# parsakhaz/multimodal-image-similarity-search

Measured on AMD Instinct MI355X. Metric: images/s CLIP-B/32 encode @ bs256; Mvec/s cosine top-10 over 10M x 512, higher is better.
Workload: dtype bf16

## Files before the change

### multimodal-image-similarity-search_amd/csrc/gemm_bf16_p160.h

```cpp
#pragma once
#include "gemm_bf16_256.h"

#define MMISS_EPI_PATCH_PIX_F32 10

#define G160_A_BYTES 20480
#define G160_W_BYTES 16384
#define G160_BUF (G160_A_BYTES + 2 * G160_W_BYTES)
#define G160_DUMP (3 * G160_BUF)
#define G160_LDS (G160_DUMP + 2048)

template <int EPI, int KT = 0>
__global__ __launch_bounds__(512, 2) void gemm160p_kernel(const __bf16* __restrict__ A, const __bf16* __restrict__ W, int M,
                                                          int N, int K, GemmEpi ep) {
    extern __shared__ __attribute__((aligned(16))) char smem[];
    typedef bf16x8 frag;
    const int tid = threadIdx.x;
    const int lane = tid & 63;
    const int wave = __builtin_amdgcn_readfirstlane(tid >> 6);
    const int wm = wave >> 2, wn = wave & 3;
    const int fr = lane & 15, fg = lane >> 4;
    const int nbm = M / 160, nbn = N >> 8;
    const int nt = KT > 0 ? KT : K / GEMM_BK;
    const int wg = xcd_remap(blockIdx.x, nbm * nbn);
    int bm, bn;
    tile_order(wg, nbm, nbn, 0, bm, bn);
    const __bf16* Ab = A + (size_t)bm * 160 * K;
    const __bf16* Wb = W + (size_t)bn * 256 * K;

    constexpr bool RESID = (EPI == MMISS_EPI_BIAS_RESID_BF16);
    constexpr bool PIX = (EPI == MMISS_EPI_PATCH_PIX_F32);
    constexpr bool PATCH = (EPI == MMISS_EPI_PATCH_F32) || PIX;
    static_assert(RESID || PATCH, "gemm160p_kernel: epilogue");
    const int r_in = lane >> 3, p = lane & 7;
    int lane_vo = (r_in * K + ((p ^ r_in) * 8)) * 2;
    __amdgpu_buffer_rsrc_t srdA = __builtin_amdgcn_make_buffer_rsrc(const_cast<__bf16*>(Ab), 0, 0x7fffffff, 0x00020000);
    __amdgpu_buffer_rsrc_t srdW = __builtin_amdgcn_make_buffer_rsrc(const_cast<__bf16*>(Wb), 0, 0x7fffffff, 0x00020000);
    const int row8 = 8 * K * 2;
    const int a_so = wave * row8;
    const int a_dst = wave * 1024;
    const int w_so = ((wave >> 1) * 64 + (wave & 1) * 16) * K * 2;
    const int w_dst = wave * 2048;
    int xa0 = a_so, xa1 = a_so + 8 * row8, xa2 = a_so + 16 * row8, xaf = a_so;
    int xw0 = w_so, xw1 = w_so + row8, xw2 = w_so + 4 * row8, xw3 = w_so + 5 * row8;
    int kstep = GEMM_BK * 2;
#define G160_X(var, expr) (RESID ? (var) : (expr))
    char* const dump = smem + G160_DUMP + wave * 256;
#define G160_BLDS(srd, so, dst) \
    __builtin_amdgcn_raw_ptr_buffer_load_lds(srd, (__attribute__((address_space(3))) void*)(dst), 16, lane_vo, so, 0, 0)
#define G160_FILL(srd, so) \
    __builtin_amdgcn_raw_ptr_buffer_load_lds(srd, (__attribute__((address_space(3))) void*)(dump), 4, lane_vo, so, 0, 0)
#define G160_STAGE_A(b2, ko)                                                                                 \
    {                                                                                                       \
        char* sl_ = smem + (b2) * G160_BUF + a_dst;                                                         \
        G160_BLDS(srdA, G160_X(xa0, a_so) + (ko), sl_);                                                     \
        G160_BLDS(srdA, G160_X(xa1, a_so + 8 * row8) + (ko), sl_ + 8 * 1024);                               \
        if (wave < 4) { G160_BLDS(srdA, G160_X(xa2, a_so + 16 * row8) + (ko), sl_ + 16 * 1024); }           \
        else { G160_FILL(srdA, G160_X(xaf, a_so) + (ko)); }                                                 \
    }
#define G160_STAGE_W(b2, nq, ko)                                                                             \
    {                                                                                                       \
        char* sl_ = smem + (b2) * G160_BUF + G160_A_BYTES + (nq) * G160_W_BYTES + w_dst;                    \
        const int so_ = G160_X((nq) ? xw2 : xw0, w_so + (nq) * 4 * row8) + (ko);                            \
        G160_BLDS(srdW, so_, sl_);                                                                          \
        G160_BLDS(srdW, G160_X(((nq) ? xw3 : xw1) + (ko), so_ + row8), sl_ + 1024);                         \
    }

    const int rblk = 16 * ep.ldo * 2;
    const int lane_vo_r = ((lane >> 2) * ep.ldo + (((lane & 3) ^ (lane >> 4)) * 8)) * 2;
#define G160_NEXT_KTILE()                                                                                    \
    if (++k2 == nt) {                                                                                       \
        if constexpr (RESID) {                                                                              \
            srdA = srdW = __builtin_amdgcn_make_buffer_rsrc(                                                \
                reinterpret_cast<uint16_t*>(ep.out) + (size_t)(bm * 160 + wm * 80) * ep.ldo + bn * 256 + wn * 64, 0, 0x7fffffff, \
                0x00020000);                                                                                \
            lane_vo = lane_vo_r;                                                                            \
            xa0 = 0; xa1 = 64; xa2 = 0; xaf = 0;                                                            \
            xw0 = rblk; xw1 = rblk + 64; xw2 = 2 * rblk; xw3 = 2 * rblk + 64;                               \
            ko2 = 0; kstep = 2 * rblk;                                                                      \
        } else { k2 = 0; ko2 = 0; }                                                                         \
    } else { ko2 += kstep; }

    u32x4 srdP = {0u, 0u, 0u, 0u};
    int pvo[3] = {0, 0, 0};
    u32x4 pa[2][6];
    int pix_S = 0, pix_tshift = 0, pix_rows = 0, pix_half = 0;
    if constexpr (PIX) {
        const uint64_t a64 = (uint64_t)A;
        srdP = u32x4{(uint32_t)a64, (uint32_t)(a64 >> 32) & 0xffffu, (uint32_t)ep.pix_bytes, 0x00020000u};
        const int S = ep.pix_S, P = ep.pix_P, G = S / P, GG = ep.p0;
        pix_S = S;
        pix_tshift = P == 32 ? 4 : 2;
        pix_rows = 64 / P;
        const int dky = P == 32 ? 0 : (p >> 2), kx = P == 32 ? p * 4 : (p & 3) * 4;
        pix_half = (P == 32 ? 1 : 2) * S * 4;
#pragma unroll
        for (int j = 0; j < 3; ++j) {
            const int q = wave + 8 * ((j == 2 && wave >= 4) ? 1 : j);
            int m = bm * 160 + q * 8 + r_in;
            m = m < ep.m_valid ? m : ep.m_valid - 1;
            const int img = m / GG, pr = m - img * GG, py = pr / G, px = pr - py * G;
            pvo[j] = (((img * 3) * S + py * P + dky) * S + px * P + kx) * 4;
        }
    }
#define G160_PIX_LOAD(set, kt)                                                                               \
    {                                                                                                       \
        const int c_ = (kt) >> pix_tshift;                                                                  \
        const int so_ = (c_ * pix_S + ((kt) - (c_ << pix_tshift)) * pix_rows) * pix_S * 4;                  \
        const int so2_ = so_ + pix_half;                                                                    \
        _Pragma("unroll") for (int j = 0; j < 3; ++j)                                                       \
            asm volatile("buffer_load_dwordx4 %0, %2, %3, %4 offen\n\tbuffer_load_dwordx4 %1, %2, %3, %5 offen" \
                         : "=&v"(pa[set][2 * j]), "=&v"(pa[set][2 * j + 1])                                 \
                         : "v"(pvo[j]), "s"(srdP), "s"(so_), "s"(so2_)                                      \
                         : "memory");                                                                       \
    }
#define G160_PIX_WRITE(set, b2, cnt)                                                                         \
    {                                                                                                       \
        asm volatile("s_waitcnt vmcnt(" #cnt ")"                                                            \
                     : "+v"(pa[set][0]), "+v"(pa[set][1]), "+v"(pa[set][2]), "+v"(pa[set][3]), "+v"(pa[set][4]), "+v"(pa[set][5]) \
                     :: "memory");                                                                          \
         \
        const int ao_ = (b2) * G160_BUF + a_dst + r_in * 128 + (((p >> 1) ^ r_in) << 4) + ((p & 1) << 3);   \
        _Pragma("unroll") for (int j = 0; j < 3; ++j) {                                                     \
            const u32x4 lo_ = pa[set][2 * j], hi_ = pa[set][2 * j + 1];                                     \
            u32x2 pl_, ph_;                                                                                 \
            pl_[0] = pack_bf16x2(__uint_as_float(lo_[0]), __uint_as_float(lo_[1]));                         \
            pl_[1] = pack_bf16x2(__uint_as_float(lo_[2]), __uint_as_float(lo_[3]));                         \
            ph_[0] = pack_bf16x2(__uint_as_float(hi_[0]), __uint_as_float(hi_[1]));                         \
            ph_[1] = pack_bf16x2(__uint_as_float(hi_[2]), __uint_as_float(hi_[3]));                         \
            if (j < 2 || wave < 4) {                                                                        \
                *reinterpret_cast<u32x2*>(smem + ao_ + j * 8 * 1024) = pl_;                                 \
                *reinterpret_cast<u32x2*>(smem + (ao_ ^ 64) + j * 8 * 1024) = ph_;                          \
            }                                                                                               \
        }                                                                                                   \
    }

    uint32_t ab[2], wb[2];
#pragma unroll
    for (int s = 0; s < 2; ++s) {
        const uint32_t sw = (((4 * s + fg) ^ (fr & 7)) << 4);
        ab[s] = (wm * 80 + fr) * 128 + sw;
        wb[s] = G160_A_BYTES + (wn * 32 + fr) * 128 + sw;
    }
    frag am[5];
    frag wq[4];
    f32x4 acc[4][5];
#pragma unroll
    for (int i = 0; i < 4; ++i)
#pragma unroll
        for (int j = 0; j < 5; ++j) acc[i][j] = f32x4{0.f, 0.f, 0.f, 0.f};

#define G160_READ(b, s)                                                                                      \
    {                                                                                                       \
        _Pragma("unroll") for (int mf = 0; mf < 5; ++mf)                                                    \
            am[mf] = *reinterpret_cast<const frag*>(smem + ab[s] + (b) * G160_BUF + mf * 2048);             \
        _Pragma("unroll") for (int i = 0; i < 4; ++i)                                                       \
            wq[i] = *reinterpret_cast<const frag*>(smem + wb[s] + (b) * G160_BUF + (i >> 1) * G160_W_BYTES + (i & 1) * 2048); \
    }
#define G160_MMA()                                                                                           \
    {                                                                                                       \
        __builtin_amdgcn_s_setprio(1);                                                                      \
        _Pragma("unroll") for (int i = 0; i < 4; ++i)                                                       \
            _Pragma("unroll") for (int mf = 0; mf < 5; ++mf)                                                \
                acc[i][mf] = __builtin_amdgcn_mfma_f32_16x16x32_bf16(wq[i], am[mf], acc[i][mf], 0, 0, 0);   \
        __builtin_amdgcn_s_setprio(0);                                                                      \
    }
#define G160_KTILE(B, B2)                                                                                    \
    {                                                                                                       \
        G160_READ(B, 0);                                                                                    \
        G160_STAGE_A(B2, ko2);                                                                              \
        p256s_late_reads_done(wm);                                                                             \
        p256s_barrier();                                                                                     \
        G160_MMA();                                                                                         \
        p256s_barrier();                                                                                     \
        G160_READ(B, 1);                                                                                    \
        G160_STAGE_W(B2, 0, ko2);                                                                           \
        G160_STAGE_W(B2, 1, ko2);                                                                           \
        p256s_late_reads_done(wm);                                                                             \
        asm volatile("s_waitcnt vmcnt(7)" ::: "memory");                                                    \
        p256s_barrier();                                                                                     \
        G160_MMA();                                                                                         \
        p256s_barrier();                                                                                     \
        G160_NEXT_KTILE();                                                                                  \
    }

#define G160_KTILE_PIX(B, B1, B2, SET)                                                                       \
    {                                                                                                       \
        G160_READ(B, 0);                                                                                    \
        G160_PIX_LOAD(SET, k2);                                                                             \
        p256s_late_reads_done(wm);                                                                             \
        p256s_barrier();                                                                                     \
        G160_MMA();                                                                                         \
        p256s_barrier();                                                                                     \
        G160_READ(B, 1);                                                                                    \
        G160_PIX_WRITE((SET) ^ 1, B1, 10);                                                                  \
        G160_STAGE_W(B2, 0, ko2);                                                                           \
        G160_STAGE_W(B2, 1, ko2);                                                                           \
        asm volatile("s_waitcnt vmcnt(10) lgkmcnt(0)" ::: "memory");                                        \
        p256s_barrier();                                                                                     \
        G160_MMA();                                                                                         \
        p256s_barrier();                                                                                     \
        G160_NEXT_KTILE();                                                                                  \
    }

    f32x4 bias[4];
    if constexpr (RESID) {
#pragma unroll
        for (int i = 0; i < 4; ++i) bias[i] = *reinterpret_cast<const f32x4*>(ep.bias + bn * 256 + wn * 64 + i * 16 + 4 * fg);
    }

    int ko2 = 0, k2 = 2;
    if constexpr (PIX) {
        G160_PIX_LOAD(0, 0);
        G160_STAGE_W(0, 0, 0);
        G160_STAGE_W(0, 1, 0);
        G160_PIX_LOAD(1, 1);
        G160_STAGE_W(1, 0, GEMM_BK * 2);
        G160_STAGE_W(1, 1, GEMM_BK * 2);
        G160_PIX_WRITE(0, 0, 14);
        ko2 = 2 * GEMM_BK * 2;
        asm volatile("s_waitcnt vmcnt(10) lgkmcnt(0)" ::: "memory");
    } else {
    G160_STAGE_A(0, 0);
    G160_STAGE_W(0, 0, 0);
    G160_STAGE_W(0, 1, 0);
    G160_STAGE_A(1, GEMM_BK * 2);
    G160_STAGE_W(1, 0, GEMM_BK * 2);
    G160_STAGE_W(1, 1, GEMM_BK * 2);
    ko2 = (nt > 2) ? 2 * GEMM_BK * 2 : 0;
    asm volatile("s_waitcnt vmcnt(7)" ::: "memory");
    }
    if constexpr (RESID) {
#pragma unroll
        for (int i = 0; i < 4; ++i) asm volatile("" : "+v"(bias[i]));
    }
    p256s_barrier();
    if (wm == 1) p256s_barrier();

    if constexpr (PIX) {
#pragma unroll 1
        for (int t = 0; t < nt; t += 6) {
            G160_KTILE_PIX(0, 1, 2, 0);
            G160_KTILE_PIX(1, 2, 0, 1);
            G160_KTILE_PIX(2, 0, 1, 0);
            G160_KTILE_PIX(0, 1, 2, 1);
            G160_KTILE_PIX(1, 2, 0, 0);
            G160_KTILE_PIX(2, 0, 1, 1);
        }
    } else {
#pragma unroll 1
    for (int t = 0; t < nt; t += 3) {
        G160_KTILE(0, 2);
        if (t + 1 < nt) G160_KTILE(1, 0);
        if (t + 2 < nt) G160_KTILE(2, 1);
    }
    }
    if (wm == 0) p256s_barrier();
    asm volatile("s_waitcnt vmcnt(0)" ::: "memory");
    p256s_barrier();
    const int free_buf = RESID ? ((nt + 2) % 3) * G160_BUF : 0;

    if constexpr (PATCH) {
        int lane_e = lane;
        asm volatile("" : "+v"(lane_e));
        const int efr = lane_e & 15, efg = lane_e >> 4;
        const int rrow = lane_e >> 3, rchunk = lane_e & 7;
        char* patch = smem + free_buf + wave * 2048;
        float* outp = reinterpret_cast<float*>(ep.out);
#pragma unroll
        for (int j = 0; j < 5; ++j) {
#pragma unroll
            for (int h = 0; h < 2; ++h) {
#pragma unroll
                for (int ii = 0; ii < 2; ++ii)
                    *reinterpret_cast<f32x4*>(patch + efr * 128 + (((ii * 4 + efg) ^ (efr & 7)) << 4)) = acc[2 * h + ii][j];
                __builtin_amdgcn_fence(__ATOMIC_RELEASE, "wavefront");
                __builtin_amdgcn_wave_barrier();
                __builtin_amdgcn_fence(__ATOMIC_ACQUIRE, "wavefront");
#pragma unroll
                for (int rh = 0; rh < 2; ++rh) {
                    const int row = rh * 8 + rrow;
                    const f32x4 v = *reinterpret_cast<const f32x4*>(patch + row * 128 + ((rchunk ^ (row & 7)) << 4));
                    const int m = bm * 160 + wm * 80 + j * 16 + row;
                    const int n = bn * 256 + wn * 64 + h * 32 + rchunk * 4;
                    if (m < ep.m_valid) {
                        const int img = m / ep.p0, pt = m - img * ep.p0;
                        const f32x4 pos = *reinterpret_cast<const f32x4*>(ep.aux + (size_t)(1 + pt) * ep.ldo + n);
                        *reinterpret_cast<f32x4*>(outp + ((size_t)img * ep.p1 + 1 + pt) * ep.ldo + n) = v + pos;
                    }
                }
                __builtin_amdgcn_wave_barrier();
            }
        }
    }
    if constexpr (RESID) {
        int lane_e = lane;
        asm volatile("" : "+v"(lane_e));
        const int efr = lane_e & 15, efg = lane_e >> 4;
        const int rrow = lane_e >> 3, rchunk = lane_e & 7;
        const __amdgpu_buffer_rsrc_t srdO = __builtin_amdgcn_make_buffer_rsrc(ep.out, 0, 0x7fffffff, 0x00020000);
        char* patch = smem + free_buf + wave * 2048;
        const int wr_off = efr * 128, wr_sw = 2 * (efr & 7);
        const int col = bn * 256 + wn * 64 + rchunk * 8;
        const int dump_row = M - 1;
        u32x2 resid[5][4];
        {
            const char* const st0 = smem + (nt % 3) * G160_BUF;
            const char* const st1 = smem + ((nt + 1) % 3) * G160_BUF;
            const int rd = efr * 64 + ((((efg >> 1) ^ (efr >> 2)) << 4) | ((efg & 1) << 3));
#pragma unroll
            for (int j = 0; j < 5; ++j)
#pragma unroll
                for (int i = 0; i < 4; ++i) {
                    const int h = i >> 1;
                    const char* piece = j == 0 ? st0 + a_dst + h * 8 * 1024
                                               : (j < 3 ? st0 : st1) + G160_A_BYTES + ((j - 1) & 1) * G160_W_BYTES + w_dst + h * 1024;
                    resid[j][i] = *reinterpret_cast<const u32x2*>(piece + (rd ^ ((i & 1) << 5)));
                }
        }
#pragma unroll
        for (int j = 0; j < 5; ++j) {
#pragma unroll
            for (int i = 0; i < 4; ++i) {
                const f32x4 v = acc[i][j] + bias[i];
                float y[4];
                y[0] = __uint_as_float(resid[j][i][0] << 16) + v[0];
                y[1] = __uint_as_float(resid[j][i][0] & 0xFFFF0000u) + v[1];
                y[2] = __uint_as_float(resid[j][i][1] << 16) + v[2];
                y[3] = __uint_as_float(resid[j][i][1] & 0xFFFF0000u) + v[3];
                u32x2 pk;
                pk[0] = pack_bf16x2(y[0], y[1]);
                pk[1] = pack_bf16x2(y[2], y[3]);
                *reinterpret_cast<u32x2*>(patch + wr_off + (((i * 4 + efg) ^ wr_sw) << 3)) = pk;
            }
            __builtin_amdgcn_fence(__ATOMIC_RELEASE, "wavefront");
            __builtin_amdgcn_wave_barrier();
            __builtin_amdgcn_fence(__ATOMIC_ACQUIRE, "wavefront");
#pragma unroll
            for (int rh = 0; rh < 2; ++rh) {
                const int row = rh * 8 + rrow;
                const u32x4 pk = *reinterpret_cast<const u32x4*>(patch + row * 128 + (((2 * rchunk) ^ (2 * (row & 7))) << 3));
                const int m = bm * 160 + wm * 80 + j * 16 + row;
                const int vo = ((m < ep.m_valid ? m : dump_row) * ep.ldo + col) * 2;
                __builtin_amdgcn_raw_buffer_store_b128(pk, srdO, vo, 0, 0);
                if (ep.stats_out) {
                    float rs = 0.f, rq = 0.f;
#pragma unroll
                    for (int e = 0; e < 4; ++e) {
                        const float a = __uint_as_float(pk[e] << 16), b = __uint_as_float(pk[e] & 0xFFFF0000u);
                        rs += a + b;
                        rq += a * a + b * b;
                    }
                    rs += __shfl_xor(rs, 1); rq += __shfl_xor(rq, 1);
                    rs += __shfl_xor(rs, 2); rq += __shfl_xor(rq, 2);
                    rs += __shfl_xor(rs, 4); rq += __shfl_xor(rq, 4);
                    if (rchunk == 0 && m < ep.m_valid) {
                        float* so = ep.stats_out + ((size_t)m * (ep.ldo >> 6) + ((bn * 256 + wn * 64) >> 6)) * 2;
                        so[0] = rs;
                        so[1] = rq;
                    }
                }
            }
            __builtin_amdgcn_wave_barrier();
        }
    }
}
#undef G160_BLDS
#undef G160_FILL
#undef G160_STAGE_A
#undef G160_STAGE_W
#undef G160_READ
#undef G160_MMA
#undef G160_KTILE
#undef G160_KTILE_PIX
#undef G160_PIX_LOAD
#undef G160_PIX_WRITE
#undef G160_NEXT_KTILE
#undef G160_X

static inline bool gemm160p_ok(int M, int N, int K) {
    if (M <= 0 || (M % 160) || N <= 0 || (N % 256) || K < 256 || (K % 128)) return false;
    if ((int64_t)M * N * 2 >= (1LL << 31) || (int64_t)160 * K * 2 >= (1LL << 31) || (int64_t)256 * K * 2 >= (1LL << 31)) return false;
    return true;
}

static int launch_gemm160p(hipStream_t st, const void* A, const void* W, const GemmEpi& ep, int M, int N, int K) {
    if (!gemm160p_ok(M, N, K)) MM_FAIL(MMISS_ERR_UNSUPPORTED, "gemm160p: M=%d N=%d K=%d", M, N, K);
    if (!ep.out || !ep.bias || ep.ldo < N || (ep.ldo % 64)) MM_FAIL(MMISS_ERR_ARG, "gemm160p: missing operand");
    const int mv = ep.m_valid < M ? ep.m_valid : M;
    const double bytes = 2.0 * ((double)mv * K + (double)N * K) + 2.0 * 2.0 * (double)mv * N;
    char pname[48];
    snprintf(pname, sizeof(pname), "gemm_bf16_bias_resid16_p160_k%d", K);
    MM_PROF(pname, st, 2.0 * mv * N * K, bytes);
#define G160_KT_CASE(KT_)                                                                                                        \
    if (K == (KT_) * GEMM_BK) {                                                                                                  \
        MM_TRY(mmiss_ensure_dyn_lds(reinterpret_cast<const void*>(&gemm160p_kernel<MMISS_EPI_BIAS_RESID_BF16, KT_>), G160_LDS)); \
        hipLaunchKernelGGL((gemm160p_kernel<MMISS_EPI_BIAS_RESID_BF16, KT_>), dim3((M / 160) * (N / 256)), dim3(512), G160_LDS, \
                           st, reinterpret_cast<const __bf16*>(A), reinterpret_cast<const __bf16*>(W), M, N, K, ep);            \
        MM_HIP(hipGetLastError());                                                                                              \
        return MMISS_OK;                                                                                                        \
    }
    G160_KT_CASE(12) G160_KT_CASE(48) G160_KT_CASE(8) G160_KT_CASE(32) G160_KT_CASE(16) G160_KT_CASE(64)
#undef G160_KT_CASE
    MM_TRY(mmiss_ensure_dyn_lds(reinterpret_cast<const void*>(&gemm160p_kernel<MMISS_EPI_BIAS_RESID_BF16>), G160_LDS));
    hipLaunchKernelGGL((gemm160p_kernel<MMISS_EPI_BIAS_RESID_BF16>), dim3((M / 160) * (N / 256)), dim3(512), G160_LDS, st, reinterpret_cast<const __bf16*>(A),
                       reinterpret_cast<const __bf16*>(W), M, N, K, ep);
    MM_HIP(hipGetLastError());
    return MMISS_OK;
}

static int launch_gemm160p_patch(hipStream_t st, const void* A, const void* W, const GemmEpi& ep, int M, int N, int K) {
    if (!gemm160p_ok(M, N, K)) MM_FAIL(MMISS_ERR_UNSUPPORTED, "gemm160p_patch: M=%d N=%d K=%d", M, N, K);
    if (!ep.out || !ep.aux || ep.p0 <= 0 || ep.p1 <= 0 || ep.ldo < N) MM_FAIL(MMISS_ERR_ARG, "gemm160p_patch: missing operand");
    const int mv = ep.m_valid < M ? ep.m_valid : M;
    MM_PROF("gemm_bf16_patch_p160", st, 2.0 * mv * N * K, 2.0 * ((double)mv * K + (double)N * K) + 4.0 * (double)mv * N);
    MM_TRY(mmiss_ensure_dyn_lds(reinterpret_cast<const void*>(&gemm160p_kernel<MMISS_EPI_PATCH_F32>), G160_LDS));
    hipLaunchKernelGGL((gemm160p_kernel<MMISS_EPI_PATCH_F32>), dim3((M / 160) * (N / 256)), dim3(512), G160_LDS, st,
                       reinterpret_cast<const __bf16*>(A), reinterpret_cast<const __bf16*>(W), M, N, K, ep);
    MM_HIP(hipGetLastError());
    return MMISS_OK;
}

static inline bool gemm160p_pix_ok(const void* pixels, int B, int S, int P, int M, int N, int K) {
    if (!(P == 16 || P == 32) || S <= 0 || (S % P) || K != 3 * P * P || !gemm160p_ok(M, N, K)) return false;
    const int G = S / P;
    if ((int64_t)B * G * G > M || ((uintptr_t)pixels & 15)) return false;
    return (int64_t)B * 3 * S * S * 4 < (1LL << 31);
}
static int launch_gemm160p_patch_pix(hipStream_t st, const void* pixels, const void* W, const GemmEpi& ep0, int B, int S, int P, int M,
                                     int N, int K) {
    if (!gemm160p_pix_ok(pixels, B, S, P, M, N, K)) MM_FAIL(MMISS_ERR_UNSUPPORTED, "gemm160p_patch_pix: B=%d S=%d P=%d M=%d N=%d K=%d", B, S, P, M, N, K);
    GemmEpi ep = ep0;
    const int G = S / P;
    if (!ep.out || !ep.aux || ep.p0 != G * G || ep.p1 <= 0 || ep.ldo < N || ep.m_valid != B * G * G)
        MM_FAIL(MMISS_ERR_ARG, "gemm160p_patch_pix: missing operand");
    ep.pix_S = S; ep.pix_P = P; ep.pix_bytes = (int)((int64_t)B * 3 * S * S * 4);
    const int mv = ep.m_valid;
    MM_PROF("gemm_bf16_patch_p160", st, 2.0 * mv * N * K, 4.0 * (double)B * 3 * S * S + 2.0 * (double)N * K + 4.0 * (double)mv * N);
    MM_TRY(mmiss_ensure_dyn_lds(reinterpret_cast<const void*>(&gemm160p_kernel<MMISS_EPI_PATCH_PIX_F32>), G160_LDS));
    hipLaunchKernelGGL((gemm160p_kernel<MMISS_EPI_PATCH_PIX_F32>), dim3((M / 160) * (N / 256)), dim3(512), G160_LDS, st,
                       reinterpret_cast<const __bf16*>(pixels), reinterpret_cast<const __bf16*>(W), M, N, K, ep);
    MM_HIP(hipGetLastError());
    return MMISS_OK;
}
```

Before: 92460.

## Pipeline residual GEMM epilogue with double-buffered patch and DPP row reductions

```diff
diff --git a/multimodal-image-similarity-search_amd/csrc/gemm_bf16_p160.h b/multimodal-image-similarity-search_amd/csrc/gemm_bf16_p160.h
--- a/multimodal-image-similarity-search_amd/csrc/gemm_bf16_p160.h
+++ b/multimodal-image-similarity-search_amd/csrc/gemm_bf16_p160.h
@@ -8,6 +8,29 @@
 #define G160_BUF (G160_A_BYTES + 2 * G160_W_BYTES)
 #define G160_DUMP (3 * G160_BUF)
 #define G160_LDS (G160_DUMP + 2048)
+
+__device__ __forceinline__ void g160_row_sum8(float& a, float& b, float& c, float& d) {
+#define G160_DPP4(ctrl)                                              \
+    "v_add_f32_dpp %0, %0, %0 " ctrl " row_mask:0xf bank_mask:0xf\n\t" \
+    "v_add_f32_dpp %1, %1, %1 " ctrl " row_mask:0xf bank_mask:0xf\n\t" \
+    "v_add_f32_dpp %2, %2, %2 " ctrl " row_mask:0xf bank_mask:0xf\n\t" \
+    "v_add_f32_dpp %3, %3, %3 " ctrl " row_mask:0xf bank_mask:0xf\n\t"
+    asm("s_nop 1\n\t" G160_DPP4("quad_perm:[1,0,3,2]") G160_DPP4("quad_perm:[2,3,0,1]") G160_DPP4("row_half_mirror")
+        : "+v"(a), "+v"(b), "+v"(c), "+v"(d));
+#undef G160_DPP4
+}
+
+__device__ __forceinline__ void g160_row_part(const u32x4& pk, float& rs, float& rq) {
+#pragma clang fp contract(off)
+    rs = 0.f;
+    rq = 0.f;
+#pragma unroll
+    for (int e = 0; e < 4; ++e) {
+        const float a = __uint_as_float(pk[e] << 16), b = __uint_as_float(pk[e] & 0xFFFF0000u);
+        rs += a + b;
+        rq += a * a + b * b;
+    }
+}
 
 template <int EPI, int KT = 0>
 __global__ __launch_bounds__(512, 2) void gemm160p_kernel(const __bf16* __restrict__ A, const __bf16* __restrict__ W, int M,
@@ -255,16 +278,15 @@
     }
     }
     if (wm == 0) p256s_barrier();
-    asm volatile("s_waitcnt vmcnt(0)" ::: "memory");
-    p256s_barrier();
-    const int free_buf = RESID ? ((nt + 2) % 3) * G160_BUF : 0;
 
     if constexpr (PATCH) {
+        asm volatile("s_waitcnt vmcnt(0)" ::: "memory");
+        p256s_barrier();
         int lane_e = lane;
         asm volatile("" : "+v"(lane_e));
         const int efr = lane_e & 15, efg = lane_e >> 4;
         const int rrow = lane_e >> 3, rchunk = lane_e & 7;
-        char* patch = smem + free_buf + wave * 2048;
+        char* patch = smem + wave * 2048;
         float* outp = reinterpret_cast<float*>(ep.out);
 #pragma unroll
         for (int j = 0; j < 5; ++j) {
@@ -297,71 +319,83 @@
         asm volatile("" : "+v"(lane_e));
         const int efr = lane_e & 15, efg = lane_e >> 4;
         const int rrow = lane_e >> 3, rchunk = lane_e & 7;
+        u32x2 resid[5][4];
+        const char* const st0 = smem + (nt % 3) * G160_BUF;
+        const char* const st1 = smem + ((nt + 1) % 3) * G160_BUF;
+        const int rd = efr * 64 + ((((efg >> 1) ^ (efr >> 2)) << 4) | ((efg & 1) << 3));
+#define G160_OLD_ROWS(j)                                                                                     \
+    _Pragma("unroll") for (int i = 0; i < 4; ++i) {                                                         \
+        const int h = i >> 1;                                                                               \
+        const char* piece = (j) == 0 ? st0 + a_dst + h * 8 * 1024                                           \
+                                     : ((j) < 3 ? st0 : st1) + G160_A_BYTES + (((j) - 1) & 1) * G160_W_BYTES + w_dst + h * 1024; \
+        resid[j][i] = *reinterpret_cast<const u32x2*>(piece + (rd ^ ((i & 1) << 5)));                       \
+    }
+        asm volatile("s_waitcnt vmcnt(7)" ::: "memory");
+        G160_OLD_ROWS(0);
+        G160_OLD_ROWS(1);
+        G160_OLD_ROWS(2);
+        p256s_barrier();
+        char* const patch = smem + ((nt + 2) % 3) * G160_BUF + wave * 4096;
+        const int wr0 = efr * 128 + ((efg ^ (2 * (efr & 7))) << 3);
+        const int wr[4] = {wr0, wr0 ^ 32, wr0 ^ 64, wr0 ^ 96};
+        const int rdp = rrow * 128 + ((rchunk ^ rrow) << 4);
+        const int row0 = bm * 160 + wm * 80, col0 = bn * 256 + wn * 64;
         const __amdgpu_buffer_rsrc_t srdO = __builtin_amdgcn_make_buffer_rsrc(ep.out, 0, 0x7fffffff, 0x00020000);
-        char* patch = smem + free_buf + wave * 2048;
-        const int wr_off = efr * 128, wr_sw = 2 * (efr & 7);
-        const int col = bn * 256 + wn * 64 + rchunk * 8;
-        const int dump_row = M - 1;
-        u32x2 resid[5][4];
-        {
-            const char* const st0 = smem + (nt % 3) * G160_BUF;
-            const char* const st1 = smem + ((nt + 1) % 3) * G160_BUF;
-            const int rd = efr * 64 + ((((efg >> 1) ^ (efr >> 2)) << 4) | ((efg & 1) << 3));
-#pragma unroll
-            for (int j = 0; j < 5; ++j)
-#pragma unroll
-                for (int i = 0; i < 4; ++i) {
-                    const int h = i >> 1;
-                    const char* piece = j == 0 ? st0 + a_dst + h * 8 * 1024
-                                               : (j < 3 ? st0 : st1) + G160_A_BYTES + ((j - 1) & 1) * G160_W_BYTES + w_dst + h * 1024;
-                    resid[j][i] = *reinterpret_cast<const u32x2*>(piece + (rd ^ ((i & 1) << 5)));
-                }
-        }
+        const int vo0 = ((row0 + rrow) * ep.ldo + col0 + rchunk * 8) * 2;
+        const int vo_dump = ((M - 1) * ep.ldo + col0 + rchunk * 8) * 2;
+        const int ostep = 8 * ep.ldo * 2;
+        const int lim = ep.m_valid - row0 - rrow;
+        const int mv = ep.m_valid < M ? ep.m_valid : M;
+        const __amdgpu_buffer_rsrc_t srdS =
+            __builtin_amdgcn_make_buffer_rsrc(ep.stats_out, 0, ep.stats_out ? mv * (ep.ldo >> 6) * 8 : 0, 0x00020000);
+        const int so0 = rchunk == 0 ? ((row0 + rrow) * (ep.ldo >> 6) + (col0 >> 6)) * 8 : (int)0x80000000u;
+        const int sstep = 8 * (ep.ldo >> 6) * 8;
+#define G160_BLOCK(j)                                                                                        \
+    _Pragma("unroll") for (int i = 0; i < 4; ++i) {                                                         \
+        const f32x4 v = acc[i][j] + bias[i];                                                                \
+        float y[4];                                                                                         \
+        y[0] = __uint_as_float(resid[j][i][0] << 16) + v[0];                                                \
+        y[1] = __uint_as_float(resid[j][i][0] & 0xFFFF0000u) + v[1];                                        \
+        y[2] = __uint_as_float(resid[j][i][1] << 16) + v[2];                                                \
+        y[3] = __uint_as_float(resid[j][i][1] & 0xFFFF0000u) + v[3];                                        \
+        u32x2 pk;                                                                                           \
+        pk[0] = pack_bf16x2(y[0], y[1]);                                                                    \
+        pk[1] = pack_bf16x2(y[2], y[3]);                                                                    \
+        *reinterpret_cast<u32x2*>(patch + ((j) & 1) * 2048 + wr[i]) = pk;                                   \
+    }
+        G160_BLOCK(0);
 #pragma unroll
         for (int j = 0; j < 5; ++j) {
-#pragma unroll
-            for (int i = 0; i < 4; ++i) {
-                const f32x4 v = acc[i][j] + bias[i];
-                float y[4];
-                y[0] = __uint_as_float(resid[j][i][0] << 16) + v[0];
-                y[1] = __uint_as_float(resid[j][i][0] & 0xFFFF0000u) + v[1];
-                y[2] = __uint_as_float(resid[j][i][1] << 16) + v[2];
-                y[3] = __uint_as_float(resid[j][i][1] & 0xFFFF0000u) + v[3];
-                u32x2 pk;
-                pk[0] = pack_bf16x2(y[0], y[1]);
-                pk[1] = pack_bf16x2(y[2], y[3]);
-                *reinterpret_cast<u32x2*>(patch + wr_off + (((i * 4 + efg) ^ wr_sw) << 3)) = pk;
-            }
             __builtin_amdgcn_fence(__ATOMIC_RELEASE, "wavefront");
             __builtin_amdgcn_wave_barrier();
             __builtin_amdgcn_fence(__ATOMIC_ACQUIRE, "wavefront");
+            u32x4 pk[2];
+#pragma unroll
+            for (int rh = 0; rh < 2; ++rh) pk[rh] = *reinterpret_cast<const u32x4*>(patch + (j & 1) * 2048 + rh * 1024 + rdp);
+            if (j == 0) { G160_BLOCK(1); }
+            if (j == 1) { G160_BLOCK(2); }
+            if (j == 2) { G160_BLOCK(3); }
+            if (j == 3) { G160_BLOCK(4); }
+            if (j == 0) {
+                asm volatile("s_waitcnt vmcnt(0)" ::: "memory");
+                G160_OLD_ROWS(3);
+                G160_OLD_ROWS(4);
+            }
+            float rs[2], rq[2];
 #pragma unroll
             for (int rh = 0; rh < 2; ++rh) {
-                const int row = rh * 8 + rrow;
-                const u32x4 pk = *reinterpret_cast<const u32x4*>(patch + row * 128 + (((2 * rchunk) ^ (2 * (row & 7))) << 3));
-                const int m = bm * 160 + wm * 80 + j * 16 + row;
-                const int vo = ((m < ep.m_valid ? m : dump_row) * ep.ldo + col) * 2;
-                __builtin_amdgcn_raw_buffer_store_b128(pk, srdO, vo, 0, 0);
-                if (ep.stats_out) {
-                    float rs = 0.f, rq = 0.f;
-#pragma unroll
-                    for (int e = 0; e < 4; ++e) {
-                        const float a = __uint_as_float(pk[e] << 16), b = __uint_as_float(pk[e] & 0xFFFF0000u);
-                        rs += a + b;
-                        rq += a * a + b * b;
-                    }
-                    rs += __shfl_xor(rs, 1); rq += __shfl_xor(rq, 1);
-                    rs += __shfl_xor(rs, 2); rq += __shfl_xor(rq, 2);
-                    rs += __shfl_xor(rs, 4); rq += __shfl_xor(rq, 4);
-                    if (rchunk == 0 && m < ep.m_valid) {
-                        float* so = ep.stats_out + ((size_t)m * (ep.ldo >> 6) + ((bn * 256 + wn * 64) >> 6)) * 2;
-                        so[0] = rs;
-                        so[1] = rq;
-                    }
-                }
+                const int k = 2 * j + rh;
+                __builtin_amdgcn_raw_buffer_store_b128(pk[rh], srdO, 8 * k < lim ? vo0 + k * ostep : vo_dump, 0, 16);
+                g160_row_part(pk[rh], rs[rh], rq[rh]);
             }
-            __builtin_amdgcn_wave_barrier();
+            g160_row_sum8(rs[0], rq[0], rs[1], rq[1]);
+#pragma unroll
+            for (int rh = 0; rh < 2; ++rh)
+                __builtin_amdgcn_raw_buffer_store_b64(u32x2{__float_as_uint(rs[rh]), __float_as_uint(rq[rh])}, srdS,
+                                                      so0 + (2 * j + rh) * sstep, 0, 0);
         }
+#undef G160_OLD_ROWS
+#undef G160_BLOCK
     }
 }
 #undef G160_BLDS
```

Result: faster. 94780, median of 6 (+2.5%).
